# WarmCongee/SDUMC

Measured on AMD Instinct MI355X. Metric: train samples/sec at MOSEI feature shapes (two-stream forward + 6-term loss + backward + Adam), higher is better.
Workload: dtype f32

## Files before the change

### include/sdumc_hip.h

```cpp
#ifndef SDUMC_HIP_H
#define SDUMC_HIP_H

#include <stddef.h>
#include <stdint.h>

#ifdef __cplusplus
extern "C" {
#endif

#define SDUMC_OK 0
#define SDUMC_EINVAL (-1)
#define SDUMC_ELAUNCH (-2)
#define SDUMC_ENOMEM (-3)

#define SDUMC_MAX_GROUPS 8
#define SDUMC_D 256
#define SDUMC_H 128
#define SDUMC_NQ 7
#define SDUMC_RNC_DIM 64
#define SDUMC_N_SITES 35

typedef struct sdumc_dropout {
  uint32_t enabled;
  uint32_t site;
// ... 415 lines not shown
  const float* src; float* dst;
  int32_t ld_src, ld_dst, rows, cols;
} sdumc_copy_seg;
int sdumc_copy2d_multi(const sdumc_copy_seg* segs, int32_t n, void* stream);
int sdumc_axpy2d(const float* src, int32_t ld_src, float* dst, int32_t ld_dst, int32_t rows, int32_t cols, void* stream);
int sdumc_copy2d(const float* src, int32_t ld_src, float* dst, int32_t ld_dst, int32_t rows, int32_t cols, void* stream);
int sdumc_fill(float* p, float v, int64_t n, void* stream);
int sdumc_rng_advance(uint32_t* dev_state, uint32_t inc, void* stream);
int sdumc_dropout_bits(const sdumc_dropout* d, int32_t streams, uint8_t* bits, void* stream);
int sdumc_dropout_bits_multi(const sdumc_dropout* d, int32_t streams, int32_t nsite, int32_t site_stride,
                             uint8_t* const* bits, void* stream);
int sdumc_dropout_bits_apply_bf16(const sdumc_dropout* d, int32_t streams, int32_t site_stride, uint8_t* const* bits,
                                  const void* x, int64_t x_rows, void* const* xd, void* stream);
int sdumc_dropout_mask(const sdumc_dropout* d, int32_t streams, float* mask, void* stream);
const char* sdumc_version(void);

typedef struct sdumc_prof_entry {
  const char* name;
  int64_t launches;
  double total_ms;
  double total_flops;
} sdumc_prof_entry;
int sdumc_profile_enable(int on);
int sdumc_profile_report(sdumc_prof_entry* out, int max_entries);

int64_t sdumc_param_count(int32_t da, int32_t dt, int32_t dv);
int64_t sdumc_param_live_count(int32_t da, int32_t dt, int32_t dv);
int32_t sdumc_param_table(int32_t da, int32_t dt, int32_t dv, char* buf, size_t buflen);

typedef struct sdumc_net_dims {
  int32_t B;
  int32_t streams;
  int32_t Ta, Tv;
  int32_t Tt[2];
  int32_t da, dt, dv;
  int32_t train;
  int32_t sample0;
  double p_frame;
  double p_mlp;
  int32_t bf16;
} sdumc_net_dims;

typedef struct sdumc_net_io {
  const float* audio;
  const float* video;
  const float* text[2];
  float* params;
  const uint32_t* rng_state;
  void* workspace;
  size_t workspace_bytes;
  float* vals;
  float* fused;
  float* rnc;
  float* text_hidden;
  float* cross_text;
  const int32_t* lengths[4];
  const void* audio_p3;
  const void* video_p3;
  const void* text_p3[2];
  const int32_t* row_map[4];
  int64_t store_rows[4];
  void* bits_next;
  int32_t bits_phase;
  size_t bits_next_bytes;
  const struct sdumc_net_dims* bits_next_dims;
  const sdumc_gather_desc* prefetch;
  int32_t prefetch_workgroups;
  void* ctx;
} sdumc_net_io;

size_t sdumc_net_bits_next_bytes(const sdumc_net_dims* d);
int sdumc_ctx_create(void** ctx);
int sdumc_ctx_destroy(void* ctx);
enum { SDUMC_OPT_CONCURRENCY = 0, SDUMC_OPT_BACKGROUND_LANE = 1, SDUMC_OPT_CHAIN_CLUSTER = 2, SDUMC_OPT_SPLIT = 3 };
int sdumc_ctx_set_option(void* ctx, int32_t option, int32_t value);

int sdumc_set_concurrency(int on);
int sdumc_set_background_lane(int on);
int sdumc_set_chain_cluster(int on);
int sdumc_chain_cluster_error_(void);
int sdumc_chain_cluster_reset_error(void);
int sdumc_chain_cluster_test_hold_(int on);
int sdumc_chain_cluster_debug_read_(uint32_t* out, int n);
int sdumc_chain_cluster_error_flag(float* flag, void* stream);
int sdumc_chain_cluster_error_merge(const float* flag, void* stream);
int sdumc_debug_marks(int on);
int sdumc_debug_marks_read(float* ms, int n);
int32_t sdumc_debug_plan_table(const sdumc_net_dims* d, char* buf, size_t buflen);
size_t sdumc_net_workspace_bytes(const sdumc_net_dims* d);
int sdumc_net_forward(const sdumc_net_dims* d, const sdumc_net_io* io, void* stream);

typedef struct sdumc_net_grads {
  const float* d_vals;
  const float* d_fused;
  const float* d_rnc;
  const float* d_text_hidden;
  const float* d_cross_text;
  float* grads;
} sdumc_net_grads;

int sdumc_net_backward(const sdumc_net_dims* d, const sdumc_net_io* io, const sdumc_net_grads* g, void* stream);
int sdumc_net_backward_phase(const sdumc_net_dims* d, const sdumc_net_io* io, const sdumc_net_grads* g, int32_t phase,
                             void* stream);
int64_t sdumc_param_early_count(int32_t da, int32_t dt, int32_t dv);

typedef struct sdumc_step_cfg {
  float weights[6];
  float temperature;
  float beta1, beta2, eps, weight_decay;
  const float* labels;
  float* adam_m;
  float* adam_v;
  float* hyper;
  float* losses;
  int32_t B_global;
  const float* ssd_global;
  const float* rnc_feats_global;
  const float* rnc_labels_global;
  int32_t rnc_row0[2];
  int32_t distill;
} sdumc_step_cfg;
#define SDUMC_DISTILL_RMSE 0
#define SDUMC_DISTILL_COSINE 1
#define SDUMC_DISTILL_KL 2

size_t sdumc_loss_workspace_bytes(const sdumc_net_dims* d, int32_t B_global);
int sdumc_loss_ssd(const sdumc_net_dims* d, const sdumc_net_io* io, float* ssd_out, void* scratch,
                   size_t scratch_bytes, void* stream);
int sdumc_dp_pack(const float* rnc, const float* labels, const float* ssd, int32_t B, int32_t rd, float* record,
                  void* stream);
size_t sdumc_dp_record_workspace_bytes(int32_t B);
int sdumc_dp_record(int32_t B, int32_t rd, const float* text_hidden, const float* cross_text, const float* fused,
                    const float* rnc, const float* labels, float* record, void* workspace, void* stream);
int sdumc_dp_unpack(const float* records, int32_t W, int32_t B, int32_t rd, float* feats, float* labels2, float* ssd,
                    void* stream);
int sdumc_loss_backward(const sdumc_net_dims* d, const sdumc_net_io* io, const sdumc_step_cfg* cfg,
                        const sdumc_net_grads* g, void* scratch, size_t scratch_bytes, void* stream);

size_t sdumc_step_workspace_bytes(const sdumc_net_dims* d);
int sdumc_train_step(const sdumc_net_dims* d, const sdumc_net_io* io, const sdumc_step_cfg* cfg, void* stream);
size_t sdumc_step_grads_offset(const sdumc_net_dims* d);

#ifdef __cplusplus
}
#endif
#endif
```

### sdumc_amd/_lib.py

```python
import ctypes as C
import os

_HERE = os.path.dirname(os.path.abspath(__file__))
LIB_PATH = os.environ.get("SDUMC_LIB") or os.path.join(_HERE, "csrc", "libsdumc_hip.so")

MAX_GROUPS = 8
D, H, NQ, RNC_DIM, N_SITES = 256, 128, 7, 64, 35
NT, NN, TN = 0, 1, 2
ACT_NONE, ACT_RELU, ACT_TANH = 0, 1, 2

c_float_p = C.c_void_p


class Dropout(C.Structure):
    _fields_ = [("enabled", C.c_uint32), ("site", C.c_uint32), ("threshold", C.c_uint32), ("scale", C.c_float),
                ("rows", C.c_uint32), ("width", C.c_uint32), ("samples", C.c_uint32), ("sample0", C.c_uint32),
                ("call0", C.c_uint32), ("stream0", C.c_uint32), ("seed_lo", C.c_uint32), ("seed_hi", C.c_uint32),
                ("dev_state", C.c_void_p), ("bits", C.c_void_p)]


class Gemm(C.Structure):
    _fields_ = [("layout", C.c_int32), ("M", C.c_int32), ("N", C.c_int32), ("K", C.c_int32),
                ("groups", C.c_int32),
                ("A", C.c_void_p * MAX_GROUPS), ("B", C.c_void_p * MAX_GROUPS),
# ... 227 lines not shown
    "sdumc_attnpool_fwd": (C.c_int, [C.POINTER(AttnPool), C.c_void_p]),
    "sdumc_attnpool_fwd_workspace_bytes_dim": (C.c_size_t, [C.c_int32, C.c_int32, C.c_int32, C.c_int32]),
    "sdumc_attnpool_bwd_workspace_bytes_dim": (C.c_size_t, [C.c_int32, C.c_int32, C.c_int32, C.c_int32]),
    "sdumc_attnpool_bwd_workspace_bytes": (C.c_size_t, [C.c_int32, C.c_int32, C.c_int32]),
    "sdumc_attnpool_bwd": (C.c_int, [C.POINTER(AttnPoolBwd), C.c_void_p]),
    "sdumc_attnpool_fwd_multi": (C.c_int, [C.POINTER(AttnPool), C.c_int32, C.c_void_p]),
    "sdumc_umca_fwd": (C.c_int, [C.POINTER(Umca), C.c_void_p]),
    "sdumc_attnpool_bwd_multi": (C.c_int, [C.POINTER(AttnPoolBwd), C.c_int32, C.c_void_p]),
    "sdumc_relu_drop_bwd": (C.c_int, [C.c_void_p, C.c_void_p, C.c_float, C.c_void_p, C.c_int64, C.c_void_p]),
    "sdumc_colsum_workspace_bytes": (C.c_size_t, [C.c_int64, C.c_int32]),
    "sdumc_colsum": (C.c_int, [C.c_void_p, C.c_int64, C.c_int32, C.c_int32, C.c_void_p, C.c_int32, C.c_void_p, C.c_void_p]),
    "sdumc_add_n": (C.c_int, [C.POINTER(C.c_void_p), C.c_int32, C.c_void_p, C.c_int64, C.c_void_p]),
    "sdumc_dropsum_bwd": (C.c_int, [C.POINTER(DropSum), C.c_void_p]),
    "sdumc_fusion_fwd": (C.c_int, [C.c_void_p, C.c_void_p, C.c_void_p, C.c_int32, C.c_void_p]),
    "sdumc_fusion_bwd": (C.c_int, [C.c_void_p, C.c_void_p, C.c_void_p, C.c_void_p, C.c_void_p, C.c_int32, C.c_void_p]),
    "sdumc_hweight_fwd": (C.c_int, [C.c_void_p, C.c_void_p, C.c_void_p, C.c_int32, C.c_void_p]),
    "sdumc_hweight_bwd": (C.c_int, [C.c_void_p, C.c_void_p, C.c_void_p, C.c_void_p, C.c_void_p, C.c_void_p, C.c_int32, C.c_float, C.c_void_p]),
    "sdumc_zpool_fwd": (C.c_int, [C.c_void_p, C.c_void_p, C.c_void_p, C.c_int32, C.c_void_p]),
    "sdumc_zpool_bwd": (C.c_int, [C.c_void_p, C.c_void_p, C.c_void_p, C.c_void_p, C.c_void_p, C.c_int32, C.c_void_p]),
    "sdumc_mse_fwd_bwd": (C.c_int, [C.c_void_p, C.c_void_p, C.c_int32, C.c_float, C.c_float, C.c_void_p, C.c_void_p, C.c_void_p]),
    "sdumc_ssd_workspace_bytes": (C.c_size_t, [C.c_int64]),
    "sdumc_ssd": (C.c_int, [C.c_void_p, C.c_void_p, C.c_int64, C.c_void_p, C.c_void_p, C.c_void_p]),
    "sdumc_rmse_bwd": (C.c_int, [C.c_void_p, C.c_void_p, C.c_int64, C.c_void_p, C.c_double, C.c_float, C.c_void_p,
                                 C.c_void_p, C.c_int32, C.c_void_p, C.c_int32, C.c_void_p]),
    "sdumc_cosine_fwd_bwd": (C.c_int, [C.c_void_p, C.c_void_p, C.c_int32, C.c_int32, C.c_int32, C.c_float, C.c_float,
                                       C.c_void_p, C.c_void_p, C.c_void_p, C.c_void_p]),
    "sdumc_kl_fwd_bwd": (C.c_int, [C.c_void_p, C.c_void_p, C.c_int32, C.c_int32, C.c_int32, C.c_float, C.c_float,
                                   C.c_void_p, C.c_void_p, C.c_void_p, C.c_void_p]),
    "sdumc_ce_fwd_bwd": (C.c_int, [C.c_void_p, C.c_void_p, C.c_int32, C.c_int32, C.c_int32, C.c_float, C.c_float,
                                   C.c_void_p, C.c_void_p, C.c_void_p, C.c_void_p]),
    "sdumc_rnc_workspace_bytes": (C.c_size_t, [C.c_int32]),
    "sdumc_rnc_fwd_bwd": (C.c_int, [C.c_void_p, C.c_void_p, C.c_int32, C.c_int32, C.c_float, C.c_float, C.c_int32,
                                    C.c_int32, C.c_void_p, C.c_void_p, C.c_void_p, C.c_void_p]),
    "sdumc_rnc_fwd_bwd_rep": (C.c_int, [C.c_void_p, C.c_void_p, C.c_int32, C.c_int32, C.c_float, C.c_float, C.c_int32,
                                        C.c_int32, C.c_void_p, C.c_void_p, C.c_void_p, C.c_void_p]),
    "sdumc_distill_workspace_bytes": (C.c_size_t, [C.c_int32]),
    "sdumc_distill_fwd_bwd": (C.c_int, [C.c_int32, C.c_float] + [C.c_void_p] * 14),
    "sdumc_rnc_dfeat_rows": (C.c_int, [C.c_void_p, C.c_int32, C.c_int32, C.c_float, C.c_float, C.c_int32, C.c_int32,
                                       C.c_void_p, C.c_void_p, C.c_void_p]),
    "sdumc_rnc_mask": (C.c_int, [C.c_void_p, C.c_int32, C.c_void_p, C.c_void_p]),
    "sdumc_adam_step": (C.c_int, [C.c_void_p, C.c_void_p, C.c_void_p, C.c_void_p, C.c_int64, C.c_void_p,
                                  C.c_float, C.c_float, C.c_float, C.c_float, C.c_float, C.c_void_p]),
    "sdumc_adam_multi": (C.c_int, [C.POINTER(AdamSeg), C.c_int32, C.c_void_p, C.c_void_p, C.c_int64, C.c_void_p,
                                   C.c_float, C.c_float, C.c_float, C.c_float, C.c_float, C.c_void_p]),
    "sdumc_copy2d": (C.c_int, [C.c_void_p, C.c_int32, C.c_void_p, C.c_int32, C.c_int32, C.c_int32, C.c_void_p]),
    "sdumc_axpy2d": (C.c_int, [C.c_void_p, C.c_int32, C.c_void_p, C.c_int32, C.c_int32, C.c_int32, C.c_void_p]),
    "sdumc_gather_pad": (C.c_int, [C.c_void_p, C.c_void_p, C.c_void_p, C.c_int32, C.c_int32, C.c_int32, C.c_void_p, C.c_void_p]),
    "sdumc_mask_apply_bf16": (C.c_int, [C.c_void_p, C.c_void_p, C.c_void_p, C.c_int64, C.c_int64, C.c_int32, C.c_float, C.c_void_p]),
    "sdumc_gemm_bf16_workspace_bytes": (C.c_size_t, [C.POINTER(GemmBf16)]),
    "sdumc_gemm_bf16_run": (C.c_int, [C.POINTER(GemmBf16), C.c_void_p]),
    "sdumc_ctx_create": (C.c_int, [C.POINTER(C.c_void_p)]),
    "sdumc_ctx_destroy": (C.c_int, [C.c_void_p]),
    "sdumc_ctx_set_option": (C.c_int, [C.c_void_p, C.c_int32, C.c_int32]),
    "sdumc_gather_pad_idx": (C.c_int, [C.c_void_p, C.c_void_p, C.c_void_p, C.c_void_p, C.c_int32, C.c_int32, C.c_int32, C.c_void_p,
                                       C.c_void_p, C.c_void_p]),
    "sdumc_gather_batch": (C.c_int, [C.POINTER(GatherBatch), C.c_int32, C.c_void_p]),
    "sdumc_fill": (C.c_int, [C.c_void_p, C.c_float, C.c_int64, C.c_void_p]),
    "sdumc_rng_advance": (C.c_int, [C.c_void_p, C.c_uint32, C.c_void_p]),
    "sdumc_dropout_bits": (C.c_int, [C.POINTER(Dropout), C.c_int32, C.c_void_p, C.c_void_p]),
    "sdumc_dropout_bits_multi": (C.c_int, [C.POINTER(Dropout), C.c_int32, C.c_int32, C.c_int32, C.POINTER(C.c_void_p), C.c_void_p]),
    "sdumc_dropout_bits_apply_bf16": (C.c_int, [C.POINTER(Dropout), C.c_int32, C.c_int32, C.POINTER(C.c_void_p), C.c_void_p, C.c_int64,
                                               C.POINTER(C.c_void_p), C.c_void_p]),
    "sdumc_dropout_mask": (C.c_int, [C.POINTER(Dropout), C.c_int32, C.c_void_p, C.c_void_p]),
    "sdumc_version": (C.c_char_p, []),
    "sdumc_layernorm_fwd": (C.c_int, [C.c_void_p] * 6 + [C.c_int64, C.c_int32, C.c_float, C.c_void_p]),
    "sdumc_layernorm_bwd_workspace_bytes": (C.c_size_t, [C.c_int64, C.c_int32]),
    "sdumc_layernorm_bwd": (C.c_int, [C.c_void_p] * 9 + [C.c_int64, C.c_int32, C.c_void_p, C.c_size_t, C.c_void_p]),
    "sdumc_softmax_fwd": (C.c_int, [C.POINTER(Softmax), C.c_void_p]),
    "sdumc_softmax_bwd": (C.c_int, [C.POINTER(Softmax), C.c_void_p, C.c_void_p]),
    "sdumc_drop_add": (C.c_int, [C.POINTER(DropAdd), C.c_void_p]),
    "sdumc_mha_workspace_bytes": (C.c_size_t, [C.POINTER(Mha), C.c_int32]),
    "sdumc_mha_forward": (C.c_int, [C.POINTER(Mha), C.c_void_p]),
    "sdumc_mha_backward": (C.c_int, [C.POINTER(Mha), C.POINTER(MhaGrads), C.c_void_p]),
    "sdumc_param_count": (C.c_int64, [C.c_int32, C.c_int32, C.c_int32]),
    "sdumc_param_live_count": (C.c_int64, [C.c_int32, C.c_int32, C.c_int32]),
    "sdumc_param_table": (C.c_int32, [C.c_int32, C.c_int32, C.c_int32, C.c_char_p, C.c_size_t]),
    "sdumc_set_concurrency": (C.c_int, [C.c_int]),
    "sdumc_set_background_lane": (C.c_int, [C.c_int]),
    "sdumc_set_chain_cluster": (C.c_int, [C.c_int]),
    "sdumc_chain_cluster_error_": (C.c_int, []),
    "sdumc_chain_cluster_reset_error": (C.c_int, []),
    "sdumc_chain_cluster_test_hold_": (C.c_int, [C.c_int]),
    "sdumc_chain_cluster_debug_read_": (C.c_int, [C.c_void_p, C.c_int]),
    "sdumc_chain_cluster_error_flag": (C.c_int, [C.c_void_p, C.c_void_p]),
    "sdumc_chain_cluster_error_merge": (C.c_int, [C.c_void_p, C.c_void_p]),
    "sdumc_debug_marks": (C.c_int, [C.c_int]),
    "sdumc_debug_marks_read": (C.c_int, [C.POINTER(C.c_float), C.c_int]),
    "sdumc_attnpool_set_v2_": (C.c_int, [C.c_int]),
    "sdumc_debug_plan_table": (C.c_int32, [C.POINTER(NetDims), C.c_char_p, C.c_size_t]),
    "sdumc_net_workspace_bytes": (C.c_size_t, [C.POINTER(NetDims)]),
    "sdumc_net_bits_next_bytes": (C.c_size_t, [C.POINTER(NetDims)]),
    "sdumc_net_forward": (C.c_int, [C.POINTER(NetDims), C.POINTER(NetIO), C.c_void_p]),
    "sdumc_net_backward": (C.c_int, [C.POINTER(NetDims), C.POINTER(NetIO), C.POINTER(NetGrads), C.c_void_p]),
    "sdumc_net_backward_phase": (C.c_int, [C.POINTER(NetDims), C.POINTER(NetIO), C.POINTER(NetGrads), C.c_int32, C.c_void_p]),
    "sdumc_param_early_count": (C.c_int64, [C.c_int32, C.c_int32, C.c_int32]),
    "sdumc_step_workspace_bytes": (C.c_size_t, [C.POINTER(NetDims)]),
    "sdumc_train_step": (C.c_int, [C.POINTER(NetDims), C.POINTER(NetIO), C.POINTER(StepCfg), C.c_void_p]),
    "sdumc_loss_workspace_bytes": (C.c_size_t, [C.POINTER(NetDims), C.c_int32]),
    "sdumc_loss_ssd": (C.c_int, [C.POINTER(NetDims), C.POINTER(NetIO), C.c_void_p, C.c_void_p, C.c_size_t, C.c_void_p]),
    "sdumc_loss_backward": (C.c_int, [C.POINTER(NetDims), C.POINTER(NetIO), C.POINTER(StepCfg), C.POINTER(NetGrads),
                                      C.c_void_p, C.c_size_t, C.c_void_p]),
    "sdumc_dp_pack": (C.c_int, [C.c_void_p, C.c_void_p, C.c_void_p, C.c_int32, C.c_int32, C.c_void_p, C.c_void_p]),
    "sdumc_dp_record_workspace_bytes": (C.c_size_t, [C.c_int32]),
    "sdumc_dp_record": (C.c_int, [C.c_int32, C.c_int32, C.c_void_p, C.c_void_p, C.c_void_p, C.c_void_p, C.c_void_p,
                                  C.c_void_p, C.c_void_p, C.c_void_p]),
    "sdumc_dp_unpack": (C.c_int, [C.c_void_p, C.c_int32, C.c_int32, C.c_int32, C.c_void_p, C.c_void_p, C.c_void_p,
                                  C.c_void_p]),
    "sdumc_step_grads_offset": (C.c_size_t, [C.POINTER(NetDims)]),
}

EXPORTS = tuple(_SIGS)


class SdumcError(RuntimeError):
    pass


_ERR = {-1: "SDUMC_EINVAL (bad argument)", -2: "SDUMC_ELAUNCH (HIP launch/runtime error)",
        -3: "SDUMC_ENOMEM (workspace too small)"}


def _load():
    if not os.path.exists(LIB_PATH):
        raise SdumcError(
            f"{LIB_PATH} not found: build it with `python -c 'import __graft_entry__ as g; g.build()'` "
            "or `make -C sdumc_amd/csrc`. sdumc_amd has no CPU or PyTorch fallback.")
    lib = C.CDLL(LIB_PATH)
    for name, (res, args) in _SIGS.items():
        if os.environ.get("SDUMC_LIB") and not hasattr(lib, name):
            continue
        fn = getattr(lib, name)
        fn.restype = res
        fn.argtypes = args
    return lib


lib = _load()


def check(rc, what=""):
    if rc != 0:
        raise SdumcError(f"{what} failed: {_ERR.get(rc, rc)}")


def current_stream():
    import torch
    return C.c_void_p(torch.cuda.current_stream().cuda_stream)


def ptr(t):
    return None if t is None else t.data_ptr()


def drop_threshold(p):
    return int(float(p) * 4294967296.0)


def make_dropout(enabled, site, p, rows, width, samples, sample0=0, call0=0, seed=0, dev_state=None):
    import numpy as np
    d = Dropout()
    d.enabled = 1 if enabled else 0
    d.site = site
    d.threshold = drop_threshold(p)
    d.scale = float(np.float32(1.0) / (np.float32(1.0) - np.float32(p)))
    d.rows, d.width, d.samples, d.sample0, d.call0 = rows, width, samples, sample0, call0
    d.seed_lo, d.seed_hi = seed & 0xFFFFFFFF, (seed >> 32) & 0xFFFFFFFF
# ... 3 lines not shown
```

### sdumc_amd/csrc/chain_cluster.hip

```cpp
#include <atomic>
#include <mutex>

#include "chain_common.h"

namespace {

constexpr int CL = 4;
constexpr int OC = D / CL;
constexpr int HC = H / CL;
constexpr int PARTC = NWV * 7 * OC;
constexpr int SPIN_CAP = 400000;
static_assert(PARTC >= NWV * 2 * H, "tail layers");

struct Cl {
  uint32_t* arrive;
  uint32_t* depart;
  int32_t* err;
  uint32_t round;
  bool hold;
  uint32_t mode;
};

__device__ __forceinline__ void st4_dev(float* p, f32x4 v) {
#pragma unroll
// ... 180 lines not shown
  __syncthreads();
  for (int u = tid; u < 3 * R * NQT * (D / 4); u += NTHR) {
    const int row = u / (D / 4), cq = u - row * (D / 4);
    const int mr = row / NQT, i = row - mr * NQT;
    const int m = mr / R, v = v0 + (mr - m * R);
    f32x4 o = {0.f, 0.f, 0.f, 0.f};
    if (v < V) {
      const int nc = f.nchunk[m];
      const float* src = f.part[m] + ((size_t)v * nc * NQT + i) * D + 4 * cq;
      const float* fac = s_fac + (mr * FOLD_MAXCHUNK) * 8 + i;
      f32x4 sum = {0.f, 0.f, 0.f, 0.f};
      for (int c0 = 0; c0 < nc; c0 += 8) {
        f32x4 pv[8];
#pragma unroll
        for (int j = 0; j < 8; ++j)
          if (c0 + j < nc) pv[j] = ld4(src + (size_t)(c0 + j) * NQT * D);
#pragma unroll
        for (int j = 0; j < 8; ++j)
          if (c0 + j < nc) sum += pv[j] * fac[(c0 + j) * 8];
      }
      o = sum;
      if (dbase.enabled) {
        DropRT od = mkdrop_rt(dbase, (uint32_t)f.site[m], NQT, D);
        od.threshold = f.threshold;
        od.scale = f.scale;
        o *= drop_mask4(od, (uint32_t)(v * NQT + i), (uint32_t)cq);
      }
      if ((mr & (CL - 1)) == member) {
        st4(f.pooled[m] + ((size_t)v * NQT + i) * D + 4 * cq, sum);
        st4(out + (((size_t)m * V + v) * NQT + i) * D + 4 * cq, o);
      }
    }
    st4(s_rows + (size_t)row * D + 4 * cq, o);
  }
#if defined(SDUMC_FOLD_DBG)
  if (SDUMC_FOLD_DBG & 1) return;
#endif
  for (int mr = 0; mr < 3 * R; ++mr) {
    const int m = mr / R, v = v0 + (mr - m * R);
    if (v >= V) continue;
    const int n = f.T[m] * NQT, per = (n + CL - 1) / CL;
    const int e0 = member * per, e1 = min(n, e0 + per);
    float* w = f.attn[m] + (size_t)v * n;
    const float* fac = s_fac + (mr * FOLD_MAXCHUNK) * 8;
    for (int e = e0 + tid; e < e1; e += 4 * NTHR) {
      float wv[4];
#pragma unroll
      for (int j = 0; j < 4; ++j)
        if (e + j * NTHR < e1) wv[j] = w[e + j * NTHR];
#pragma unroll
      for (int j = 0; j < 4; ++j) {
        const int ee = e + j * NTHR;
        if (ee < e1) {
          const int t = ee / NQT, i = ee - t * NQT;
          w[ee] = wv[j] * fac[(t >> 6) * 8 + i];
        }
      }
    }
  }
}

template <int ROWS>
__device__ __forceinline__ void lds_selfcheck(const float* lds_rows, const float* src, int width, int row0, int nrows, uint32_t* dbg, int tag) {
  if (!dbg) return;
  const int q = width >> 2;
  for (int u = threadIdx.x; u < ROWS * q; u += NTHR) {
    const int r = u / q, c = u - r * q;
    if (row0 + r >= nrows) continue;
    const f32x4 l = ld4(lds_rows + r * width + 4 * c);
    const f32x4 g = ld4(src + (int64_t)(row0 + r) * width + 4 * c);
    if (__float_as_uint(l[0]) != __float_as_uint(g[0]) || __float_as_uint(l[1]) != __float_as_uint(g[1]) ||
        __float_as_uint(l[2]) != __float_as_uint(g[2]) || __float_as_uint(l[3]) != __float_as_uint(g[3])) {
      const uint32_t idx = atomicAdd(dbg, 1u);
      if (idx < 20) {
        uint32_t* rec = dbg + 8 + 12 * idx;
        rec[0] = blockIdx.x; rec[1] = threadIdx.x; rec[2] = (uint32_t)tag; rec[3] = (uint32_t)(r * width + 4 * c);
#pragma unroll
        for (int k = 0; k < 4; ++k) { rec[4 + k] = __float_as_uint(l[k]); rec[8 + k] = __float_as_uint(g[k]); }
      }
    }
  }
}

template <int ROWS, int I, int O, class Epi, class Hook>
__device__ __forceinline__ void cxm_run(CRing& ring, const float* in_lds, int ld_in, const float* __restrict__ M, int ldm, float* part,
                                        Epi&& epi, Hook&& hook) {
  constexpr int RSv = ROWS >= 14 ? 2 : 1;
  using G = CGeom<I, O, RSv>;
  constexpr int OG = G::OG, S = G::S, MW = G::MW, WAVES = G::WAVES, IW = G::IW, ITER = G::ITER;
  constexpr int RG = ROWS / RSv;
  static_assert(ROWS % RSv == 0 && RG <= 7, "rows per group");
  static_assert(RSv * WAVES * RG * O <= PARTC, "partial-sum area too small");
  const int tid = threadIdx.x, lane = tid & 63, wave = tid >> 6;
  const int grp = wave / MW, wg = wave % MW;
  const int sq = lane / OG, cg = lane % OG;
  f32x4 acc[RG];
#pragma unroll
  for (int r = 0; r < RG; ++r) acc[r] = f32x4{0.f, 0.f, 0.f, 0.f};
  if (wg < WAVES) {
    const int i0 = wg * IW + 4 * sq;
    const float* mp = M + (size_t)i0 * ldm + 4 * cg;
    const float* xin = in_lds + grp * RG * ld_in + i0;
    static_for<ITER>([&](auto jc) {
      constexpr int j = decltype(jc)::value, sl = (j % 4) * 4;
#pragma unroll
      for (int r = 0; r < RG; ++r) {
        const f32x4 x = ld4(xin + r * ld_in + j * 4 * S);
        static_for<4>([&](auto ec) {
          constexpr int e = decltype(ec)::value;
          const uint4 u = ring.w[sl + e];
          acc[r] += f32x4{__uint_as_float(u.x), __uint_as_float(u.y), __uint_as_float(u.z), __uint_as_float(u.w)} * x[e];
        });
      }
      __builtin_amdgcn_sched_barrier(0);
      if constexpr (j + 4 < ITER) cxm_load<I, O, RSv, j % 4>(ring, mp, j + 4, ldm);
    });
#pragma unroll
    for (int r = 0; r < RG; ++r)
#pragma unroll
      for (int c = 0; c < 4; ++c) {
        acc[r][c] += __shfl_xor(acc[r][c], 32, 64);
        acc[r][c] += __shfl_xor(acc[r][c], 16, 64);
        if constexpr (S == 8) acc[r][c] += __shfl_xor(acc[r][c], 8, 64);
      }
  }
  hook();
  if (wg < WAVES && sq == 0) {
#pragma unroll
    for (int r = 0; r < RG; ++r) st4(part + ((grp * WAVES + wg) * RG + r) * O + 4 * cg, acc[r]);
  }
  __syncthreads();
  for (int u = tid; u < ROWS * (O / 4); u += NTHR) {
    const int r = u / (O / 4), cq = u - r * (O / 4);
    const int g = r / RG, rr = r - g * RG;
    f32x4 v = ld4(part + ((g * WAVES) * RG + rr) * O + 4 * cq);
#pragma unroll
    for (int ww = 1; ww < WAVES; ++ww) v += ld4(part + ((g * WAVES + ww) * RG + rr) * O + 4 * cq);
    epi(r, 4 * cq, v);
  }
  __syncthreads();
}

#define TR(k) do { if (a.cl_trace && blockIdx.x == 0 && threadIdx.x == 0) a.cl_trace[k] = wall_clock64(); } while (0)

#define CL_PROLOGUE()                                                                                          \
  __shared__ int s_bail;                                                                                       \
  const int cluster = blockIdx.x % ncl, member = blockIdx.x / ncl;                                             \
  const int V = a.V, v0 = cluster * R, tid = threadIdx.x, lane = tid & 63, wave = tid >> 6;                    \
  const int coff = member * OC;                                                                                \
  Cl cl{a.cl_flags + cluster * 64, a.cl_flags + cluster * 64 + 32, a.cl_err, 0u, a.cl_test_hold == 1 && blockIdx.x == 0, (uint32_t)a.cl_mode};                              \
  if (tid == 0) s_bail = 0;                                                                                    \
  (void)lane; (void)wave

typedef float WT;
#define PF(I_, O_, ptr, ldm) cxm_prefetch<I_, O_, 1>(ring, ptr, ldm)
#define PF14(I_, O_, ptr, ldm) cxm_prefetch<I_, O_, 2>(ring, ptr, ldm)

template <int R>
__device__ __forceinline__ void chain_fwd_a_cl_body(const sdumc_chain_args a, const int ncl) {
  extern __shared__ __attribute__((aligned(16))) float sm[];
  float* part = sm;
  float* s_hpre = part + PARTC;
  float* s_u1 = s_hpre + 3 * R * D;
  float* s_u = s_u1 + 3 * R * D;
  float* s_att1 = s_u + 3 * R * D;
  float* s_att2 = s_att1 + R * D;
  float* s_alpha = s_att2 + R * D;
  float* s_qin = s_alpha + R * 4;
  float* s_q = s_qin + 7 * R * D;
  float* s_bias = s_q + 7 * R * D;
  CL_PROLOGUE();
  TR(0);
  const int64_t VD = (int64_t)V * D;
  {
    const float* bsrc[18] = {a.umlp0_b[0], a.umlp0_b[1], a.umlp0_b[2], a.umlp3_b[0], a.umlp3_b[1], a.umlp3_b[2], a.att0_b, a.att3_b,
                             a.query_b[0], a.query_b[1], a.query_b[2], a.query_b[3], a.query_b[4], a.query_b[5], a.query_b[6],
                             a.caq_b[0], a.caq_b[1], a.caq_b[2]};
    for (int u = tid; u < 18 * (D / 4); u += NTHR) st4(s_bias + 4 * u, ld4(bsrc[u / (D / 4)] + 4 * (u % (D / 4))));
  }
  const DropRT dbase = drop_resolve(a.drop);
  CRing ring;
  if (a.cl_mode & 2) __builtin_amdgcn_fence(__ATOMIC_ACQUIRE, "agent");
  if (a.cl_mode & 8)
    for (int i = 0; i < 8; ++i) __builtin_amdgcn_s_sleep(127);
  PF(D, OC, a.umlp0_w[0] + coff, D);
  if (a.cl_mode & 16) cxm_selfcheck<D, OC, 1>(ring, a.umlp0_w[0] + coff, D, a.cl_dbg);
  if (a.fra.part[0]) fold_combine<R, 1>(a.fra, a.hpre, s_hpre, s_qin, v0, V, member, dbase);
  else for (int m = 0; m < 3; ++m) load_rows<R>(s_hpre + m * R * D, a.hpre + m * VD, D, D, v0, V);
  __syncthreads();
  TR(11);
  if ((a.cl_mode & 64) && !a.fra.part[0])
    for (int m = 0; m < 3; ++m) lds_selfcheck<R>(s_hpre + m * R * D, a.hpre + m * VD, D, v0, V, a.cl_dbg, 10 + m);
#pragma unroll 1
  for (int m = 0; m < 3; ++m) {
    const DropRT dr = mkdrop_rt(dbase, 6 + 2 * m, 1, D);
    float* dst = a.u1 + m * VD + (int64_t)v0 * D;
    auto epi = [&](int r, int col, f32x4 v) {
      col += coff;
      if (v0 + r < V) st4_dev(dst + (int64_t)r * D + col, fwd_val(v, s_bias + m * D, col, true, dr, (uint32_t)(v0 + r)));
    };
    cxm_run<R, D, OC>(ring, s_hpre + m * R * D, D, a.umlp0_w[m] + coff, D, part, epi,
                                [&] { PF(D, OC, (m < 2 ? a.umlp0_w[m + 1] : a.umlp3_w[0]) + coff, D); });
  }
  TR(1);
  if ((a.cl_mode & 64) && !a.fra.part[0])
    for (int m = 0; m < 3; ++m) lds_selfcheck<R>(s_hpre + m * R * D, a.hpre + m * VD, D, v0, V, a.cl_dbg, 20 + m);
  cl_sync(cl, &s_bail);
  TR(2);
  for (int m = 0; m < 3; ++m) reload_rows<R>(s_u1 + m * R * D, D, a.u1 + m * VD, D, D, v0, V);
  __syncthreads();
#pragma unroll 1
  for (int m = 0; m < 3; ++m) {
// ... 367 lines not shown
  reload_rows<R>(s_e1, D, a.d_e1, D, D, v0, V);
  __syncthreads();
#pragma unroll 1
  for (int blk = member; blk < 14; blk += CL) {
    float* dst = a.d_h + (int64_t)v0 * NQ * H;
    const int boff = blk * OC;
    auto epi = [&](int r, int col, f32x4 v) {
      col += boff;
      if (v0 + r < V) st4_dev(dst + (int64_t)r * NQ * H + col, v + ld4(s_dh + r * NQ * H + col));
    };
    cxm_run<R, D, OC>(ring, s_e1, D, a.catt0_w + boff, NQ * H, part, epi, [&] {
      if (blk + CL < 14) PF(D, OC, a.catt0_w + boff + CL * OC, NQ * H);
      else PF14(H, OC, a.cmlp3_w[0] + coff, D);
    });
  }
  TR(3);
  cl_sync(cl, &s_bail);
  TR(4);
  reload_rows<R>(s_dh, NQ * H, a.d_h, NQ * H, NQ * H, v0, V);
  __syncthreads();
#pragma unroll 1
  for (int m = 0; m < 3; ++m) {
    float* s_dcm = s_dc + m * NQ * R * H;
    for (int u = tid; u < R * NQ * (H / 4); u += NTHR) {
      const int ri = u / (H / 4), c = 4 * (u - ri * (H / 4)), r = ri / NQ;
      const bool live = v0 + r < V;
      f32x4 cm = {0.f, 0.f, 0.f, 0.f}, g = ld4(s_dh + ri * H + c);
      if (live) cm = ld4(a.c + ((int64_t)m * VQ + (int64_t)v0 * NQ + ri) * H + c);
      part[u] = dot4(g, cm);
      g = g * s_alpha[r * 4 + m];
      if (m == 1 && a.g_cross_text && live) g += ld4(a.g_cross_text + ((int64_t)v0 * NQ + ri) * H + c);
      g = mask_val(g, cm, sc);
      st4(s_dcm + ri * H + c, g);
      if (live && wr) st4(a.d_c + ((int64_t)m * VQ + (int64_t)v0 * NQ + ri) * H + c, g);
    }
    __syncthreads();
    for (int r = wave; r < R; r += NWV) {
      float s = 0.f;
      for (int k = lane; k < NQ * (H / 4); k += 64) s += part[r * NQ * (H / 4) + k];
      s = wave_sum(s);
      if (lane == 0 && v0 + r < V && wr) a.d_alpha[(int64_t)(v0 + r) * 3 + m] = s;
    }
    __syncthreads();
  }
#pragma unroll 1
  for (int m = 0; m < 3; ++m) {
    float* dst = a.d_c1 + ((int64_t)m * VQ + (int64_t)v0 * NQ) * D;
    const float* y = s_c1 + m * NQ * R * D;
    auto epi = [&](int r, int col, f32x4 v) {
      col += coff;
      if (v0 * NQ + r < V * NQ) st4_dev(dst + (int64_t)r * D + col, mask_val(v, ld4(y + r * D + col), sc));
    };
    cxm_run<NQ * R, H, OC>(ring, s_dc + m * NQ * R * H, H, a.cmlp3_w[m] + coff, D, part, epi, [&] {
      if (m < 2) PF14(H, OC, a.cmlp3_w[m + 1] + coff, D);
      else PF14(D, OC, a.cmlp0_w[0] + coff, D);
    });
  }
  TR(5);
  cl_sync(cl, &s_bail);
  TR(6);
  cl_exit(cl);
  for (int m = 0; m < 3; ++m) reload_rows<NQ * R>(s_c1 + m * NQ * R * D, D, a.d_c1 + (int64_t)m * VQ * D, D, D, v0 * NQ, V * NQ);
  __syncthreads();
#pragma unroll 1
  for (int m = 0; m < 3; ++m) {
    float* dst = a.d_ca_out + ((int64_t)m * VQ + (int64_t)v0 * NQ) * D;
    auto epi = [&](int r, int col, f32x4 v) {
      col += coff;
      if (v0 * NQ + r < V * NQ) st4(dst + (int64_t)r * D + col, v);
    };
    cxm_run<NQ * R, D, OC>(ring, s_c1 + m * NQ * R * D, D, a.cmlp0_w[m] + coff, D, part, epi,
                                     [&] { if (m < 2) PF14(D, OC, a.cmlp0_w[m + 1] + coff, D); });
  }
  TR(31);
}
template <int R>
__global__ __launch_bounds__(NTHR) void chain_bwd_b_cl_kernel(const sdumc_chain_args a, const int ncl) { chain_bwd_b_cl_body<R>(a, ncl); }

template <int R>
__device__ __forceinline__ void chain_bwd_a_cl_body(const sdumc_chain_args a, const int ncl) {
  extern __shared__ __attribute__((aligned(16))) float sm[];
  float* part = sm;
  float* s_x = part + PARTC;
  float* s_dq = s_x + 3 * NQ * R * D;
  float* s_dqin = s_dq + NQ * R * D;
  float* s_u = s_dqin + NQ * R * D;
  float* s_du = s_u + 3 * R * D;
  float* s_a2 = s_du + 3 * R * D;
  float* s_a1 = s_a2 + R * D;
  float* s_u1 = s_a1 + R * D;
  float* s_small = s_u1 + 3 * R * D;
  CL_PROLOGUE();
  TR(0);
  const int64_t VD = (int64_t)V * D, VQ = (int64_t)V * NQ;
  const float sc = a.relu_scale;
  const bool wr = member == 0;
  float* s_alpha = s_small;
  float* s_dalpha = s_small + 4 * R;

  CRing ring;
  PF14(D, OC, a.caq_w[0] + coff, D);
  load_rows<R>(s_u, a.u, 3 * D, 3 * D, v0, V);
  load_rows<R>(s_a2, a.att2, D, D, v0, V);
  load_rows<R>(s_a1, a.att1, D, D, v0, V);
  for (int m = 0; m < 3; ++m) load_rows<R>(s_u1 + m * R * D, a.u1 + m * VD, D, D, v0, V);
  if (a.dq_part[0]) {
    for (int u = tid; u < 3 * R * NQ * (D / 4); u += NTHR) {
      const int row = u / (D / 4), cq = u - row * (D / 4);
      const int mr = row / NQ, i = row - mr * NQ;
      const int m = mr / R, v = v0 + (mr - m * R);
      f32x4 sum = {0.f, 0.f, 0.f, 0.f};
      if (v < V) {
        const int nc = a.dq_nchunk[m];
        const float* src = a.dq_part[m] + ((size_t)v * nc * NQ + i) * D + 4 * cq;
        for (int c0 = 0; c0 < nc; c0 += 8) {
          f32x4 pv[8];
#pragma unroll
          for (int j = 0; j < 8; ++j)
            if (c0 + j < nc) pv[j] = ld4(src + (size_t)(c0 + j) * NQ * D);
#pragma unroll
          for (int j = 0; j < 8; ++j)
            if (c0 + j < nc) sum += pv[j];
        }
        if ((mr & (CL - 1)) == member) st4(a.d_qp + (((size_t)m * V + v) * NQ + i) * D + 4 * cq, sum);
      }
      st4(s_x + (size_t)row * D + 4 * cq, sum);
    }
  } else {
    for (int m = 0; m < 3; ++m) load_rows<NQ * R>(s_x + m * NQ * R * D, a.d_qp + (int64_t)m * VQ * D, D, D, v0 * NQ, V * NQ);
  }
  for (int u = tid; u < R * 3; u += NTHR) {
    const int r = u / 3, j = u - 3 * r;
    s_alpha[r * 4 + j] = v0 + r < V ? a.alpha[(int64_t)(v0 + r) * 3 + j] : 0.f;
    s_dalpha[r * 4 + j] = v0 + r < V ? a.d_alpha[(int64_t)(v0 + r) * 3 + j] : 0.f;
  }
  __syncthreads();
#pragma unroll 1
  for (int m = 0; m < 3; ++m) {
    auto epi = [&](int r, int col, f32x4 v) {
      col += coff;
      if (m > 0) v += ld4(s_dq + r * D + col);
      st4(s_dq + r * D + col, v);
    };
    cxm_run<NQ * R, D, OC>(ring, s_x + m * NQ * R * D, D, a.caq_w[m] + coff, D, part, epi,
                                     [&] { if (m < 2) PF14(D, OC, a.caq_w[m + 1] + coff, D); else PF(D, OC, a.query_w[0] + coff, D); });
  }
  for (int u = tid; u < R * NQ * (OC / 4); u += NTHR) {
    const int ri = u / (OC / 4), c = coff + 4 * (u - ri * (OC / 4)), r = ri / NQ, i = ri - r * NQ;
    f32x4 g = ld4(s_dq + ri * D + c);
    const bool live = v0 + r < V;
    if (i == 5 && a.g_text_hidden && live) g += ld4(a.g_text_hidden + (int64_t)(v0 + r) * D + c);
    f32x4 y = {0.f, 0.f, 0.f, 0.f};
    if (live) y = ld4(a.q + ((int64_t)(v0 + r) * NQ + i) * D + c);
    g = mask_val(g, y, sc);
    if (live) st4_dev(a.d_q + ((int64_t)(v0 + r) * NQ + i) * D + c, g);
  }
  TR(1);
  cl_sync(cl, &s_bail);
  TR(2);
  reload_rows<R>(s_dq, NQ * D, a.d_q, NQ * D, NQ * D, v0, V);
  __syncthreads();
#pragma unroll 1
  for (int i = 0; i < 7; ++i) {
    float* dst = a.d_qin + i * VD + (int64_t)v0 * D;
    auto epi = [&](int r, int col, f32x4 v) {
      col += coff;
      if (v0 + r < V) st4_dev(dst + (int64_t)r * D + col, v);
    };
    cxm_run<R, D, OC>(ring, s_dq + i * D, NQ * D, a.query_w[i] + coff, D, part, epi,
                                [&] { PF(D, OC, (i < 6 ? a.query_w[i + 1] : a.att3_w) + coff, D); });
  }
  TR(3);
  cl_sync(cl, &s_bail);
  TR(4);
  for (int i = 0; i < 7; ++i) reload_rows<R>(s_dqin + i * R * D, D, a.d_qin + i * VD, D, D, v0, V);
  __syncthreads();
  for (int u = tid; u < R * (D / 4); u += NTHR) {
    const int r = u / (D / 4), c = 4 * (u - r * (D / 4));
    const f32x4 df = ld4(s_dqin + (0 * R + r) * D + c), dfat = ld4(s_dqin + (1 * R + r) * D + c),
                dftv = ld4(s_dqin + (2 * R + r) * D + c), dfav = ld4(s_dqin + (3 * R + r) * D + c);
    const f32x4 ga = df + dfat + dfav, gt = df + dfat + dftv, gv = df + dftv + dfav;
    const float aa = s_alpha[r * 4], at = s_alpha[r * 4 + 1], av = s_alpha[r * 4 + 2];
    st4(s_du + r * 3 * D + c, ga * aa + ld4(s_dqin + (4 * R + r) * D + c));
    st4(s_du + r * 3 * D + D + c, gt * at + ld4(s_dqin + (5 * R + r) * D + c));
    st4(s_du + r * 3 * D + 2 * D + c, gv * av + ld4(s_dqin + (6 * R + r) * D + c));
    part[(r * 3 + 0) * (D / 4) + (c >> 2)] = dot4(ga, ld4(s_u + r * 3 * D + c));
    part[(r * 3 + 1) * (D / 4) + (c >> 2)] = dot4(gt, ld4(s_u + r * 3 * D + D + c));
    part[(r * 3 + 2) * (D / 4) + (c >> 2)] = dot4(gv, ld4(s_u + r * 3 * D + 2 * D + c));
  }
  __syncthreads();
  for (int p = wave; p < 3 * R; p += NWV) {
    const float s = wave_sum(part[p * (D / 4) + lane]);
    if (lane == 0) {
      const int r = p / 3, j = p - 3 * r;
      const float da = s_dalpha[r * 4 + j] + s;
      s_dalpha[r * 4 + j] = da;
      if (v0 + r < V && wr) a.d_alpha[(int64_t)(v0 + r) * 3 + j] = da;
    }
  }
  __syncthreads();
  for (int u = tid; u < R * (D / 4); u += NTHR) {
    const int r = u / (D / 4), c = 4 * (u - r * (D / 4));
    f32x4 g = ld4(a.fc_att_w + c) * s_dalpha[r * 4] + ld4(a.fc_att_w + D + c) * s_dalpha[r * 4 + 1] +
              ld4(a.fc_att_w + 2 * D + c) * s_dalpha[r * 4 + 2];
    g = mask_val(g, ld4(s_a2 + r * D + c), sc);
    st4(s_a2 + r * D + c, g);
    if (v0 + r < V && wr) st4(a.d_att2 + (int64_t)(v0 + r) * D + c, g);
  }
  __syncthreads();
  {
    float* dst = a.d_att1 + (int64_t)v0 * D;
    auto epi = [&](int r, int col, f32x4 v) {
      col += coff;
      if (v0 + r < V) st4_dev(dst + (int64_t)r * D + col, mask_val(v, ld4(s_a1 + r * D + col), sc));
    };
    cxm_run<R, D, OC>(ring, s_a2, D, a.att3_w + coff, D, part, epi, [&] { PF(D, OC, a.att0_w + member * OC, 3 * D); });
  }
  TR(5);
  cl_sync(cl, &s_bail);
  TR(6);
  reload_rows<R>(s_a1, D, a.d_att1, D, D, v0, V);
  __syncthreads();
#pragma unroll 1
  for (int blk = member; blk < 12; blk += CL) {
    float* dst = a.d_u + (int64_t)v0 * 3 * D;
    const int boff = blk * OC;
    auto epi = [&](int r, int col, f32x4 v) {
      col += boff;
      if (v0 + r < V) st4_dev(dst + (int64_t)r * 3 * D + col, mask_val(v + ld4(s_du + r * 3 * D + col), ld4(s_u + r * 3 * D + col), sc));
    };
    cxm_run<R, D, OC>(ring, s_a1, D, a.att0_w + boff, 3 * D, part, epi, [&] {
      if (blk + CL < 12) PF(D, OC, a.att0_w + boff + CL * OC, 3 * D);
      else PF(D, OC, a.umlp3_w[0] + coff, D);
    });
  }
  TR(7);
  cl_sync(cl, &s_bail);
  TR(8);
  reload_rows<R>(s_du, 3 * D, a.d_u, 3 * D, 3 * D, v0, V);
  __syncthreads();
#pragma unroll 1
  for (int m = 0; m < 3; ++m) {
    float* dst = a.d_u1 + m * VD + (int64_t)v0 * D;
    const float* y = s_u1 + m * R * D;
    auto epi = [&](int r, int col, f32x4 v) {
      col += coff;
      if (v0 + r < V) st4_dev(dst + (int64_t)r * D + col, mask_val(v, ld4(y + r * D + col), sc));
    };
    cxm_run<R, D, OC>(ring, s_du + m * D, 3 * D, a.umlp3_w[m] + coff, D, part, epi,
                                [&] { PF(D, OC, (m < 2 ? a.umlp3_w[m + 1] : a.umlp0_w[0]) + coff, D); });
  }
  TR(9);
  cl_sync(cl, &s_bail);
  TR(10);
  cl_exit(cl);
  for (int m = 0; m < 3; ++m) reload_rows<R>(s_u1 + m * R * D, D, a.d_u1 + m * VD, D, D, v0, V);
  __syncthreads();
#pragma unroll 1
  for (int m = 0; m < 3; ++m) {
    float* dst = a.d_hpre + m * VD + (int64_t)v0 * D;
    auto epi = [&](int r, int col, f32x4 v) {
      col += coff;
      if (v0 + r < V) st4(dst + (int64_t)r * D + col, v);
    };
    cxm_run<R, D, OC>(ring, s_u1 + m * R * D, D, a.umlp0_w[m] + coff, D, part, epi,
                                [&] { if (m < 2) PF(D, OC, a.umlp0_w[m + 1] + coff, D); });
  }
  TR(31);
}
template <int R>
__global__ __launch_bounds__(NTHR) void chain_bwd_a_cl_kernel(const sdumc_chain_args a, const int ncl) { chain_bwd_a_cl_body<R>(a, ncl); }

#undef PF
#undef PF14
#undef CL_PROLOGUE

template <int R> constexpr size_t smem_fwd_a() { return sizeof(float) * (PARTC + 11 * R * D + 4 * R + 14 * R * D + 18 * D); }
template <int R> constexpr size_t smem_fwd_b() { return sizeof(float) * (PARTC + 3 * NQ * R * D + 3 * NQ * R * H + R * NQ * H + R * D + 2 * R * H + R * RD + 12 * R + 4 * D + 4 * H + 2 * RD); }
template <int R> constexpr size_t smem_bwd_b() { return sizeof(float) * (PARTC + 2 * R * RD + R * H + 2 * R * NQ * H + R * H + R * D + 3 * NQ * R * H + 3 * NQ * R * D + 24 * R); }
template <int R> constexpr size_t smem_bwd_a() { return sizeof(float) * (PARTC + 3 * NQ * R * D + 2 * NQ * R * D + 6 * R * D + 2 * R * D + 3 * R * D + 8 * R); }

template <class K>
int set_smem(K kernel, size_t bytes) {
  return hipFuncSetAttribute(reinterpret_cast<const void*>(kernel), hipFuncAttributeMaxDynamicSharedMemorySize, (int)bytes) == hipSuccess
             ? SDUMC_OK : SDUMC_ELAUNCH;
}

struct ClusterDev {
  std::mutex mu;
  uint32_t* flags = nullptr;
  int32_t* err = nullptr;
  unsigned long long* trace = nullptr;
  uint32_t* dbg = nullptr;
  bool tracing = false;
  hipEvent_t done = nullptr;
  hipStream_t last = nullptr;
  bool any = false;
  bool multi = false;
  int cus = 0;
  int attr = 0;
  int test_hold = 0;
};
ClusterDev g_cl[16];
constexpr int kMaxClusters = 128;

ClusterDev* cluster_dev() {
  int dev = 0;
  if (hipGetDevice(&dev) != hipSuccess || dev < 0 || dev >= 16) return nullptr;
  ClusterDev& d = g_cl[dev];
  std::lock_guard<std::mutex> lk(d.mu);
  if (!d.flags) {
    int cus = 0;
    if (hipDeviceGetAttribute(&cus, hipDeviceAttributeMultiprocessorCount, dev) != hipSuccess) return nullptr;
    uint32_t* f = nullptr;
    if (hipMalloc(&f, (kMaxClusters * 64 + 64 + 256 + 256) * sizeof(uint32_t)) != hipSuccess) return nullptr;
    if (hipMemset(f, 0, (kMaxClusters * 64 + 64 + 256 + 256) * sizeof(uint32_t)) != hipSuccess) return nullptr;
    d.trace = reinterpret_cast<unsigned long long*>(f + kMaxClusters * 64 + 64);
    d.dbg = f + kMaxClusters * 64 + 64 + 256;
    if (hipEventCreateWithFlags(&d.done, hipEventDisableTiming) != hipSuccess) return nullptr;
    d.err = reinterpret_cast<int32_t*>(f + kMaxClusters * 64);
    d.cus = cus;
    d.flags = f;
  }
  return &d;
}

}

namespace { std::atomic<int> g_cluster_on{-1}; }
extern "C" int sdumc_set_chain_cluster(int on) {
  g_cluster_on.store(on ? 1 : 0);
  return SDUMC_OK;
}
namespace {
template <int R>
bool cluster_prepare(ClusterDev* d) {
  std::lock_guard<std::mutex> lk(d->mu);
  if (d->attr == 0) {
    d->attr = -1;
    if (set_smem(chain_fwd_a_cl_kernel<R>, 158 * 1024) || set_smem(chain_fwd_b_cl_kernel<R>, smem_fwd_b<R>()) ||
        set_smem(chain_bwd_b_cl_kernel<R>, smem_bwd_b<R>()) || set_smem(chain_bwd_a_cl_kernel<R>, smem_bwd_a<R>()))
      return false;
    int n[4] = {0, 0, 0, 0};
    if (hipOccupancyMaxActiveBlocksPerMultiprocessor(&n[0], chain_fwd_a_cl_kernel<R>, NTHR, smem_fwd_a<R>()) != hipSuccess ||
        hipOccupancyMaxActiveBlocksPerMultiprocessor(&n[1], chain_fwd_b_cl_kernel<R>, NTHR, smem_fwd_b<R>()) != hipSuccess ||
        hipOccupancyMaxActiveBlocksPerMultiprocessor(&n[2], chain_bwd_b_cl_kernel<R>, NTHR, smem_bwd_b<R>()) != hipSuccess ||
        hipOccupancyMaxActiveBlocksPerMultiprocessor(&n[3], chain_bwd_a_cl_kernel<R>, NTHR, smem_bwd_a<R>()) != hipSuccess)
      return false;
    if (n[0] < 1 || n[1] < 1 || n[2] < 1 || n[3] < 1) return false;
    d->attr = 1;
  }
  return d->attr == 1;
}
}

extern "C" int sdumc_chain_cluster_ok_(int V) {
  if (g_cluster_on.load() < 0) { const char* e = getenv("SDUMC_CHAIN_CLUSTER"); g_cluster_on.store(e ? (atoi(e) ? 1 : 0) : 1); }
  if (!g_cluster_on.load()) return 0;
  return sdumc_chain_cluster_fits_(V);
}
extern "C" int sdumc_chain_cluster_fits_(int V) {
  if (V <= 0) return 0;
  ClusterDev* d = cluster_dev();
  if (!d) return 0;
  const int ncl = (V + 1) / 2;
  if (!(ncl <= kMaxClusters && ncl * CL <= d->cus)) return 0;
  return cluster_prepare<2>(d) ? 1 : 0;
}

extern "C" int sdumc_chain_cluster_launch_(const sdumc_chain_args* ap, int which, void* stream) {
  if (!ap || ap->V <= 0 || which < 0 || which > 3) return SDUMC_EINVAL;
  if (!sdumc_chain_cluster_fits_(ap->V)) return 1;
  constexpr int R = 2;
  ClusterDev* d = cluster_dev();
  if (!d) return SDUMC_ELAUNCH;
  sdumc_chain_args a = *ap;
  a.cl_test_hold = d->test_hold;
  a.cl_flags = d->flags;
  a.cl_err = d->err;
  a.cl_trace = d->tracing ? d->trace + 32 * which : nullptr;
  a.w_bf16 = 0;
  a.cl_mode = 0;
  a.cl_dbg = d->dbg;
  const int ncl = (a.V + R - 1) / R;
  const dim3 grid(ncl * CL), blk(NTHR);
  hipStream_t st = as_stream(stream);
  std::lock_guard<std::mutex> lk(d->mu);
  if (d->any && d->last != st) {
    if (!d->multi) {
      d->multi = true;
      if (hipEventRecord(d->done, d->last) != hipSuccess) {
        (void)hipGetLastError();
        if (hipDeviceSynchronize() != hipSuccess) return SDUMC_ELAUNCH;
      }
    }
    if (hipStreamWaitEvent(st, d->done, 0) != hipSuccess) return SDUMC_ELAUNCH;
  }
  const size_t smem_a = (a.cl_mode & 32) ? (size_t)158 * 1024 : smem_fwd_a<R>();
  {
    switch (which) {
      case 0: hipLaunchKernelGGL(chain_fwd_a_cl_kernel<R>, grid, blk, smem_a, st, a, ncl); break;
      case 1: hipLaunchKernelGGL(chain_fwd_b_cl_kernel<R>, grid, blk, smem_fwd_b<R>(), st, a, ncl); break;
      case 2: hipLaunchKernelGGL(chain_bwd_b_cl_kernel<R>, grid, blk, smem_bwd_b<R>(), st, a, ncl); break;
      default: hipLaunchKernelGGL(chain_bwd_a_cl_kernel<R>, grid, blk, smem_bwd_a<R>(), st, a, ncl); break;
    }
  }
  SDUMC_CHECK_LAUNCH();
  if (d->multi && hipEventRecord(d->done, st) != hipSuccess) return SDUMC_ELAUNCH;
  d->last = st;
  d->any = true;
  return SDUMC_OK;
}

extern "C" int sdumc_chain_cluster_forget_stream_(void* stream) {
  for (int dev = 0; dev < 16; ++dev) {
    ClusterDev& d = g_cl[dev];
    std::lock_guard<std::mutex> lk(d.mu);
    if (d.any && d.last == as_stream(stream)) {
      if (hipStreamSynchronize(d.last) != hipSuccess) return SDUMC_ELAUNCH;
      d.any = false;
      d.last = nullptr;
    }
  }
  return SDUMC_OK;
}

extern "C" const int32_t* sdumc_chain_cluster_err_ptr_() {
  int dev = 0;
  if (hipGetDevice(&dev) != hipSuccess || dev < 0 || dev >= 16) return nullptr;
  return g_cl[dev].err;
}

extern "C" int sdumc_chain_cluster_reset_error(void) {
  ClusterDev* d = cluster_dev();
  if (!d) return SDUMC_ELAUNCH;
  if (hipDeviceSynchronize() != hipSuccess) return SDUMC_ELAUNCH;
  if (hipMemset(d->flags, 0, (kMaxClusters * 64 + 64) * sizeof(uint32_t)) != hipSuccess) return SDUMC_ELAUNCH;
  return SDUMC_OK;
}
namespace {
__global__ void cl_err_flag_kernel(const int32_t* err, float* flag) { flag[0] = (err && *err != 0) ? 1.f : 0.f; }
__global__ void cl_err_merge_kernel(int32_t* err, const float* flag) {
  if (flag[0] != 0.f) *err = 1;
}
}
extern "C" int sdumc_chain_cluster_error_flag(float* flag, void* stream) {
  if (!flag) return SDUMC_EINVAL;
  ClusterDev* d = cluster_dev();
  if (!d) return SDUMC_ELAUNCH;
  hipLaunchKernelGGL(cl_err_flag_kernel, dim3(1), dim3(1), 0, as_stream(stream), d->err, flag);
// ... 58 lines not shown
```

Baseline: 51110.

## Alias stage-A backward LDS buffers to fit two workgroups per CU

Stage A backward cluster kernel now reuses the d_qp staging area for the late buffers (dqin, du, att2, att1, u1), which shrinks its LDS footprint so two workgroups can sit on one CU. The att/u1 row loads move after the caq loop, and the weight-prefetch hook in that loop runs after the partial-sum store behind a scheduling barrier. Launch bounds gain a minimum-blocks hint, and an occupancy query entry point is added. This risks more register pressure from the launch bound and ordering hazards from the aliasing, and a cluster kernel that relies on co-resident spinning workgroups may see its scheduling change.

Result: no change. 51090 (-0.0%).

```diff
diff --git a/include/sdumc_hip.h b/include/sdumc_hip.h
--- a/include/sdumc_hip.h
+++ b/include/sdumc_hip.h
@@ -521,6 +521,7 @@
 int sdumc_chain_cluster_reset_error(void);
 int sdumc_chain_cluster_test_hold_(int on);
 int sdumc_chain_cluster_debug_read_(uint32_t* out, int n);
+int sdumc_chain_cluster_occupancy_(int which);
 int sdumc_chain_cluster_error_flag(float* flag, void* stream);
 int sdumc_chain_cluster_error_merge(const float* flag, void* stream);
 int sdumc_debug_marks(int on);
diff --git a/sdumc_amd/_lib.py b/sdumc_amd/_lib.py
--- a/sdumc_amd/_lib.py
+++ b/sdumc_amd/_lib.py
@@ -333,6 +333,7 @@
     "sdumc_chain_cluster_reset_error": (C.c_int, []),
     "sdumc_chain_cluster_test_hold_": (C.c_int, [C.c_int]),
     "sdumc_chain_cluster_debug_read_": (C.c_int, [C.c_void_p, C.c_int]),
+    "sdumc_chain_cluster_occupancy_": (C.c_int, [C.c_int]),
     "sdumc_chain_cluster_error_flag": (C.c_int, [C.c_void_p, C.c_void_p]),
     "sdumc_chain_cluster_error_merge": (C.c_int, [C.c_void_p, C.c_void_p]),
     "sdumc_debug_marks": (C.c_int, [C.c_int]),
diff --git a/sdumc_amd/csrc/chain_cluster.hip b/sdumc_amd/csrc/chain_cluster.hip
--- a/sdumc_amd/csrc/chain_cluster.hip
+++ b/sdumc_amd/csrc/chain_cluster.hip
@@ -286,7 +286,7 @@
   }
 }
 
-template <int ROWS, int I, int O, class Epi, class Hook>
+template <int ROWS, int I, int O, bool LATE_HOOK = false, class Epi, class Hook>
 __device__ __forceinline__ void cxm_run(CRing& ring, const float* in_lds, int ld_in, const float* __restrict__ M, int ldm, float* part,
                                         Epi&& epi, Hook&& hook) {
   constexpr int RSv = ROWS >= 14 ? 2 : 1;
@@ -328,10 +328,14 @@
         if constexpr (S == 8) acc[r][c] += __shfl_xor(acc[r][c], 8, 64);
       }
   }
-  hook();
+  if constexpr (!LATE_HOOK) hook();
   if (wg < WAVES && sq == 0) {
 #pragma unroll
     for (int r = 0; r < RG; ++r) st4(part + ((grp * WAVES + wg) * RG + r) * O + 4 * cg, acc[r]);
+  }
+  if constexpr (LATE_HOOK) {
+    __builtin_amdgcn_sched_barrier(0);
+    hook();
   }
   __syncthreads();
   for (int u = tid; u < ROWS * (O / 4); u += NTHR) {
@@ -865,14 +869,15 @@
   extern __shared__ __attribute__((aligned(16))) float sm[];
   float* part = sm;
   float* s_x = part + PARTC;
-  float* s_dq = s_x + 3 * NQ * R * D;
-  float* s_dqin = s_dq + NQ * R * D;
-  float* s_u = s_dqin + NQ * R * D;
-  float* s_du = s_u + 3 * R * D;
+  float* s_dqin = s_x;
+  float* s_du = s_dqin + NQ * R * D;
   float* s_a2 = s_du + 3 * R * D;
   float* s_a1 = s_a2 + R * D;
   float* s_u1 = s_a1 + R * D;
-  float* s_small = s_u1 + 3 * R * D;
+  static_assert(NQ * R * D + 3 * R * D + 2 * R * D + 3 * R * D <= 3 * NQ * R * D, "the late buffers must fit the d_qp area");
+  float* s_dq = s_x + 3 * NQ * R * D;
+  float* s_u = s_dq + NQ * R * D;
+  float* s_small = s_u + 3 * R * D;
   CL_PROLOGUE();
   TR(0);
   const int64_t VD = (int64_t)V * D, VQ = (int64_t)V * NQ;
@@ -884,9 +889,6 @@
   CRing ring;
   PF14(D, OC, a.caq_w[0] + coff, D);
   load_rows<R>(s_u, a.u, 3 * D, 3 * D, v0, V);
-  load_rows<R>(s_a2, a.att2, D, D, v0, V);
-  load_rows<R>(s_a1, a.att1, D, D, v0, V);
-  for (int m = 0; m < 3; ++m) load_rows<R>(s_u1 + m * R * D, a.u1 + m * VD, D, D, v0, V);
   if (a.dq_part[0]) {
     for (int u = tid; u < 3 * R * NQ * (D / 4); u += NTHR) {
       const int row = u / (D / 4), cq = u - row * (D / 4);
@@ -925,8 +927,8 @@
       if (m > 0) v += ld4(s_dq + r * D + col);
       st4(s_dq + r * D + col, v);
     };
-    cxm_run<NQ * R, D, OC>(ring, s_x + m * NQ * R * D, D, a.caq_w[m] + coff, D, part, epi,
-                                     [&] { if (m < 2) PF14(D, OC, a.caq_w[m + 1] + coff, D); else PF(D, OC, a.query_w[0] + coff, D); });
+    cxm_run<NQ * R, D, OC, true>(ring, s_x + m * NQ * R * D, D, a.caq_w[m] + coff, D, part, epi,
+                                           [&] { if (m < 2) PF14(D, OC, a.caq_w[m + 1] + coff, D); else PF(D, OC, a.query_w[0] + coff, D); });
   }
   for (int u = tid; u < R * NQ * (OC / 4); u += NTHR) {
     const int ri = u / (OC / 4), c = coff + 4 * (u - ri * (OC / 4)), r = ri / NQ, i = ri - r * NQ;
@@ -938,6 +940,9 @@
     g = mask_val(g, y, sc);
     if (live) st4_dev(a.d_q + ((int64_t)(v0 + r) * NQ + i) * D + c, g);
   }
+  load_rows<R>(s_a2, a.att2, D, D, v0, V);
+  load_rows<R>(s_a1, a.att1, D, D, v0, V);
+  for (int m = 0; m < 3; ++m) load_rows<R>(s_u1 + m * R * D, a.u1 + m * VD, D, D, v0, V);
   TR(1);
   cl_sync(cl, &s_bail);
   TR(2);
@@ -1052,7 +1057,7 @@
   TR(31);
 }
 template <int R>
-__global__ __launch_bounds__(NTHR) void chain_bwd_a_cl_kernel(const sdumc_chain_args a, const int ncl) { chain_bwd_a_cl_body<R>(a, ncl); }
+__global__ __launch_bounds__(NTHR, 4) void chain_bwd_a_cl_kernel(const sdumc_chain_args a, const int ncl) { chain_bwd_a_cl_body<R>(a, ncl); }
 
 #undef PF
 #undef PF14
@@ -1061,7 +1066,8 @@
 template <int R> constexpr size_t smem_fwd_a() { return sizeof(float) * (PARTC + 11 * R * D + 4 * R + 14 * R * D + 18 * D); }
 template <int R> constexpr size_t smem_fwd_b() { return sizeof(float) * (PARTC + 3 * NQ * R * D + 3 * NQ * R * H + R * NQ * H + R * D + 2 * R * H + R * RD + 12 * R + 4 * D + 4 * H + 2 * RD); }
 template <int R> constexpr size_t smem_bwd_b() { return sizeof(float) * (PARTC + 2 * R * RD + R * H + 2 * R * NQ * H + R * H + R * D + 3 * NQ * R * H + 3 * NQ * R * D + 24 * R); }
-template <int R> constexpr size_t smem_bwd_a() { return sizeof(float) * (PARTC + 3 * NQ * R * D + 2 * NQ * R * D + 6 * R * D + 2 * R * D + 3 * R * D + 8 * R); }
+template <int R> constexpr size_t smem_bwd_a() { return sizeof(float) * (PARTC + 3 * NQ * R * D + NQ * R * D + 3 * R * D + 8 * R); }
+static_assert(smem_bwd_a<2>() <= 80 * 1024, "two workgroups of stage A backward per CU");
 
 template <class K>
 int set_smem(K kernel, size_t bytes) {
@@ -1082,6 +1088,7 @@
   bool multi = false;
   int cus = 0;
   int attr = 0;
+  int occ[4] = {0, 0, 0, 0};
   int test_hold = 0;
 };
 ClusterDev g_cl[16];
@@ -1131,6 +1138,7 @@
         hipOccupancyMaxActiveBlocksPerMultiprocessor(&n[3], chain_bwd_a_cl_kernel<R>, NTHR, smem_bwd_a<R>()) != hipSuccess)
       return false;
     if (n[0] < 1 || n[1] < 1 || n[2] < 1 || n[3] < 1) return false;
+    for (int k = 0; k < 4; ++k) d->occ[k] = n[k];
     d->attr = 1;
   }
   return d->attr == 1;
@@ -1149,6 +1157,13 @@
   const int ncl = (V + 1) / 2;
   if (!(ncl <= kMaxClusters && ncl * CL <= d->cus)) return 0;
   return cluster_prepare<2>(d) ? 1 : 0;
+}
+
+extern "C" int sdumc_chain_cluster_occupancy_(int which) {
+  if (which < 0 || which > 3) return -1;
+  ClusterDev* d = cluster_dev();
+  if (!d || !cluster_prepare<2>(d)) return 0;
+  return d->occ[which];
 }
 
 extern "C" int sdumc_chain_cluster_launch_(const sdumc_chain_args* ap, int which, void* stream) {
```
